# legend-exp/LegendDSP.jl

Measured on NVIDIA B200. Metric: waveforms/sec for dsp_icpc (8192-sample), higher is better.
Workload: dtype f64

## Files before the change

legenddsp.jl_b200/csrc/lgdsp_icpc_split.cuh:

```cuda

constexpr int TTG_LEN = TT_LEN;
constexpr int AUX_LEN = 16;
enum { AX_M = 0, AX_EMAX = 1, AX_YMAX = 2, AX_THR = 3 , AX_POS = 8 , AX_BAD = 13  };

enum { K1R_BLS = 0, K1R_BLSS, K1R_BLSX, K1R_MX , K1R_MN, K1R_SLEN, K1R_SS, K1R_SQ,
       K1R_TLS, K1R_TLSS, K1R_TLSX, K1R_TLBAD, K1R_YMAX, K1R_N };

constexpr int K1_XS = 0;
constexpr int K1_MASK = K1_XS + 2 * MAXN * 2;
constexpr int K1_RED = K1_MASK + 5 * NWORDS * 4;
constexpr int K1_IRED = K1_MASK;
constexpr int K1_BAR = K1_RED + K1R_N * NWARP * 8;
constexpr int TILE_LD = 9;
constexpr int K1_TILE = K1_BAR + 16;
constexpr int K1_TOTAL = K1_TILE + NWARP * 32 * TILE_LD * 8;
static_assert(4 * (K1_TOTAL + 1024) <= 233472, "four CTAs per SM");

template <typename SAMPLE, unsigned GMASK>
__global__ void __launch_bounds__(NT, 4)
icpc_prefix_kernel(const __grid_constant__ IcpcDev P, const SAMPLE* __restrict__ wf, long long n_events, long long ld,
                   const double* __restrict__ bl_ext, long long bl_stride, double bl_div, double* __restrict__ ttg,
                   double* __restrict__ auxg, double* __restrict__ rows)
{
    extern __shared__ __align__(128) unsigned char smem[];
// ... 271 lines not shown
                    uint32_t word = (uint32_t)(mbt << lane);
                    if (lane > 0) word |= (uint32_t)(up >> (33 - lane));
                    uint32_t* M = masks + t * NWORDS;
                    const int w = (CH * wid) + lane;
                    if (w < NWORDS) M[w] = word;
                    if (lane == 31 && w + 1 < NWORDS) M[w + 1] = (uint32_t)(mbt >> 1);
                }
            }
            const double ya = wmax_d(cvalid > 0 ? fmax(fabs(ylo), fabs(yhi)) : 0.0);
            red_put(red, K1R_YMAX, wid, lane, ya);
        }
        {
            double tl_S = 0, tl_SS = 0, tl_SX = 0;
            bool bad = lean;
            double cref = 0.0, cinv = 0.0, clog = 0.0;
            const int ntail = P.tail_until - P.tail_from + 1;
            const int q = lean ? 0 : (ntail + NT - 1) / NT;
            const int ia = P.tail_from + tid * q, ib = min(ia + q - 1, P.tail_until);
            int wcat = 3;
            double c_run = 0.0, cinv_run = 0.0;
            int xref = 0;
            if (q > 0) {
                const int mfl = (int)floor(fmin(fmax(m, -2.0e9), 2.0e9));
                int dmx = 0;
                bool nonpos = false;
                xref = ia <= ib ? (int)xs[ia] : 0;
#pragma unroll 2
                for (int idx = ia; idx <= ib; ++idx) {
                    const int xv = (int)xs[idx];
                    nonpos |= xv <= mfl;
                    dmx = max(dmx, abs(xv - xref));
                }
                int cat = 0;
                if (ia <= ib) {
                    c_run = u2d((uint32_t)xref) - m;
                    cinv_run = 1.0 / c_run;
                    const double au = (double)dmx * cinv_run;
                    cat = (nonpos || !(c_run > 0.0) || au > 0.125) ? 3 : (au > 0.015625 ? 2 : (au > 0.0009765625 ? 1 : 0));
                }
                wcat = __reduce_max_sync(FULL, cat);
            }
            if (wcat < 3) {
                const double clog_run = ia <= ib ? log_d(c_run) : 0.0;
#pragma unroll 1
                for (int idx = ia; idx <= ib; ++idx) {
                    const double u = (double)((int)xs[idx] - xref) * cinv_run;
                    double lg;
                    if (wcat == 0) {
                        double pl = fma(u, 1.0 / 5.0, -1.0 / 4.0);
                        pl = fma(u, pl, 1.0 / 3.0); pl = fma(u, pl, -1.0 / 2.0); pl = fma(u, pl, 1.0);
                        lg = fma(u, pl, clog_run);
                    } else if (wcat == 1) {
                        const double u2 = u * u, u4 = u2 * u2;
                        const double a0 = fma(-1.0 / 2.0, u, 1.0), a1 = fma(-1.0 / 4.0, u, 1.0 / 3.0), a2 = fma(-1.0 / 6.0, u, 1.0 / 5.0),
                                     a3 = fma(-1.0 / 8.0, u, 1.0 / 7.0);
                        const double b0 = fma(a1, u2, a0), b1 = fma(a3, u2, a2);
                        const double c0 = fma(b1, u4, b0);
                        lg = fma(u, fma(u4 * u4, 1.0 / 9.0, c0), clog_run);
                    } else {
                        lg = clog_run + log1p_small(u);
                    }
                    const double X = t_first + (double)idx * dt;
                    tl_S += lg;
                    tl_SS = fma(lg, lg, tl_SS);
                    tl_SX = fma(X, lg, tl_SX);
                }
            } else {
#pragma unroll 1
                for (int i = 0; i < q; ++i) {
                    const int idx = ia + i;
                    const bool act = idx <= ib;
                    const double w = act ? u2d(xs[idx]) - m : cref;
                    const bool pos = w > 0.0;
                    if (act && !pos) bad = true;
                    const double u = (w - cref) * cinv, au = fabs(u);
                    const bool use = act && pos;
                    int cat = 0;
                    if (use) cat = !(cref > 0.0) || au > 0.125 ? 3 : (au > 0.015625 ? 2 : (au > 0.0009765625 ? 1 : 0));
                    const int wcat = __reduce_max_sync(FULL, cat);
                    double lg;
                    if (wcat == 0) {
                        double pl = fma(u, 1.0 / 5.0, -1.0 / 4.0);
                        pl = fma(u, pl, 1.0 / 3.0); pl = fma(u, pl, -1.0 / 2.0); pl = fma(u, pl, 1.0);
                        lg = fma(u, pl, clog);
                    } else if (wcat == 1) {
                        const double u2 = u * u, u4 = u2 * u2;
                        const double a0 = fma(-1.0 / 2.0, u, 1.0), a1 = fma(-1.0 / 4.0, u, 1.0 / 3.0), a2 = fma(-1.0 / 6.0, u, 1.0 / 5.0),
                                     a3 = fma(-1.0 / 8.0, u, 1.0 / 7.0);
                        const double b0 = fma(a1, u2, a0), b1 = fma(a3, u2, a2);
                        const double c0 = fma(b1, u4, b0);
                        lg = fma(u, fma(u4 * u4, 1.0 / 9.0, c0), clog);
                    } else {
                        lg = clog + log1p_small(u);
                        if (cat == 3) {
                            lg = log_d(w);
                            cref = w; cinv = 1.0 / w; clog = lg;
                        }
                    }
                    if (use) {
                        const double X = t_first + (double)idx * dt;
                        tl_S += lg;
                        tl_SS = fma(lg, lg, tl_SS);
                        tl_SX = fma(X, lg, tl_SX);
                    }
                }
            }
            tl_S = wsum_d(tl_S); tl_SS = wsum_d(tl_SS); tl_SX = wsum_d(tl_SX);
            const bool anybad = __any_sync(FULL, bad);
            if (lane == 0) {
                red[K1R_TLS * NWARP + wid] = tl_S; red[K1R_TLSS * NWARP + wid] = tl_SS;
                red[K1R_TLSX * NWARP + wid] = tl_SX; red[K1R_TLBAD * NWARP + wid] = anybad ? 1.0 : 0.0;
            }
        }
        __syncthreads();

        double* ax = auxg + e * AUX_LEN;
        double* ro = rows + e * LGDSP_NCOL;
        if (wid < 5) {
            int pos = -1, mult = 0;
            if ((G & LGDSP_GROUP_TIMING) && !(lean && wid != 1)) resolve_runs(masks + wid * NWORDS, P.tx_min_n, lane, pos, mult);
            if (lane == 0) { ax[AX_POS + wid] = (double)pos; ax[AX_THR + wid] = thr[wid == 0 ? 0 : wid == 1 ? 1 : wid == 2 ? 2 : wid == 3 ? 3 : 4]; }
        } else if (wid == 5) {
            const double blS = red_sum(red, K1R_BLS), blSS = red_sum(red, K1R_BLSS), blSX = red_sum(red, K1R_BLSX);
            const double tlS = red_sum(red, K1R_TLS), tlSS = red_sum(red, K1R_TLSS), tlSX = red_sum(red, K1R_TLSX);
            const double tlbad = red_sum(red, K1R_TLBAD);
            if (lane < 2) {
                const double sY = lane == 0 ? blS : tlS;
                const double sYY = lane == 0 ? blSS : tlSS;
                const double sXY = lane == 0 ? t_first * blS + dt * blSX : tlSX;
                const Stats st = stats_finalize(lane == 0 ? P.bl_inv_n : P.tail_inv_n, lane == 0 ? P.bl_sX : P.tail_sX,
                                                lane == 0 ? P.bl_sXX : P.tail_sXX, sY, sYY, sXY);
                const double bad = wrapped ? CUDART_NAN : 0.0;
                if (lane == 0) {
                    ro[LGDSP_COL_blmean] = st.mean + bad; ro[LGDSP_COL_blsigma] = st.sigma + bad;
                    ro[LGDSP_COL_blslope] = st.slope + bad; ro[LGDSP_COL_bloffset] = st.offset + bad;
                    ro[LGDSP_COL_qc_label] = -1.0 + bad;
                    ro[LGDSP_COL_e_max] = e_max + bad; ro[LGDSP_COL_e_min] = e_min + bad;
                    ro[LGDSP_COL_n_sat_low] = (double)nlow + bad; ro[LGDSP_COL_n_sat_high] = (double)nhigh + bad;
                    ro[LGDSP_COL_n_sat_low_cons] = (double)cons_low + bad; ro[LGDSP_COL_n_sat_high_cons] = (double)cons_high + bad;
                } else {
                    const bool ok = tlbad == 0.0;
                    ro[LGDSP_COL_tail_mean] = (ok ? st.mean : 0.0) + bad; ro[LGDSP_COL_tail_sigma] = (ok ? st.sigma : 0.0) + bad;
                    ro[LGDSP_COL_tail_tau] = (ok ? div_rn(-1.0, st.slope) : 0.0) + bad;
                }
            }
        } else if (wid == 6) {
            const double Ymax = red_max(red, K1R_YMAX);
            if (lane == 0) { ax[AX_M] = m; ax[AX_EMAX] = e_max; ax[AX_YMAX] = Ymax; ax[AX_BAD] = wrapped ? 1.0 : 0.0; }
        }
        __syncthreads();
    }
}

constexpr int NT2 = 256;
constexpr int NW2 = NT2 / 32;
static_assert(NT2 == NT && NW2 == NWARP, "the extract kernel shares the block-reduction helpers and the 33-sample chunking");
enum { MK_T0 = 0, MK_T0INV, MK_CUR, MK_PILE, MK_N };
enum { K2R_PZS = 0, K2R_PZSS, K2R_PZSX, K2R_E104, K2R_E104N, K2R_E313, K2R_E313N, K2R_C535, K2R_CET, K2R_SGMAX, K2R_SGS, K2R_SGSS,
       K2R_CMAX0, K2R_CMAX1, K2R_CMAX2, K2R_CMAX3, K2R_CARG0, K2R_CARG1, K2R_CARG2, K2R_CARG3, K2R_E535, K2R_ETMAX, K2R_ETARG, K2R_N };
constexpr int K2_NTYPE = 5;
constexpr int K2_TT = 0;
constexpr int K2_MASK = K2_TT + TT_LEN * 8;
constexpr int K2_RED = K2_MASK + MK_N * NWORDS * 4;
constexpr int K2_STASH = K2_RED + K2R_N * NW2 * 8;
constexpr int K2_ROW = K2_STASH + LGDSP_MAX_DNI * 8;
constexpr int K2_AUX = K2_ROW + 64 * 8;
constexpr int K2_SGG = K2_AUX + AUX_LEN * 8;
constexpr int K2_FLAG = K2_SGG + 24 * 8;
constexpr int K2_BAR = K2_FLAG + NT2;
constexpr int K2_TOTAL = K2_BAR + 16;
static_assert(3 * (K2_TOTAL + 1024) <= 233472, "three CTAs per SM");

template <unsigned GMASK>
__global__ void __launch_bounds__(NT2, 3)
icpc_extract_kernel(const __grid_constant__ IcpcDev P, const double* __restrict__ ttg, const double* __restrict__ auxg,
                    long long n_events, int write_cz_zeros, double* __restrict__ rows)
{
    extern __shared__ __align__(128) unsigned char smem[];
    double* TT = reinterpret_cast<double*>(smem + K2_TT);
    uint32_t* masks = reinterpret_cast<uint32_t*>(smem + K2_MASK);
    double* red = reinterpret_cast<double*>(smem + K2_RED);
    double* stash = reinterpret_cast<double*>(smem + K2_STASH);
    double* row = reinterpret_cast<double*>(smem + K2_ROW);
    double* aux = reinterpret_cast<double*>(smem + K2_AUX);
    double (*sgg)[8] = reinterpret_cast<double (*)[8]>(smem + K2_SGG);
    unsigned char* flagb = smem + K2_FLAG;
    uint64_t* bar = reinterpret_cast<uint64_t*>(smem + K2_BAR);

    const int tid = threadIdx.x, lane = tid & 31, wid = tid >> 5;
    const int n = P.n;
    const uint32_t tt_bytes = (uint32_t)(n + 2) * 8u;
    const double t_first = P.t_first, dt = P.dt;
    const unsigned G = GMASK ? GMASK : P.groups;
    const double* A_int = P.dni_A;
    const double* A_sig = P.dni_A + LGDSP_MAX_DNI * 4;

    if (tid == 0) {
        mbar_init(bar, 1);
        fence_mbar_init();
    }
    if (tid < TT_LEN - 2 - n) TT[n + 2 + tid] = 0.0;
    if (tid < 24) sgg[tid >> 3][tid & 7] = P.sg[tid >> 3].gg[tid & 7];
    __syncthreads();
    auto sg_at = [&](int f, int j) -> double {
        return (P.sg[f].n_taps + 1 <= 8) ? sg_eval8(TT, sgg[f], j) : sg_eval(TT, P.sg[f].gg, P.sg[f].n_taps, j);
    };
    const int i0 = tid * CH;
    const int nsg = P.sg[0].nout;
    const bool want_cur = (G & LGDSP_GROUP_CURRENT) != 0, want_intr = (G & LGDSP_GROUP_INTRACE) != 0;

    uint32_t it = 0;
    for (long long e = blockIdx.x; e < n_events; e += gridDim.x, ++it) {
        if (tid == 0) {
            fence_proxy_async();
            mbar_expect_tx(bar, tt_bytes);
            tma_load_1d(TT, ttg + e * TTG_LEN, tt_bytes, bar);
            if (e + gridDim.x < n_events) tma_prefetch_l2(ttg + (e + gridDim.x) * TTG_LEN, tt_bytes);
        }
#pragma unroll
        for (int q = 0; q < MK_N; ++q) masks[q * NWORDS + tid] = 0u;
        if (tid < AUX_LEN) aux[tid] = auxg[e * AUX_LEN + tid];
        mbar_wait(bar, it & 1u);

        const bool lean = (G & LGDSP_GROUP_LEAN) != 0;
        const TrapDev& T5 = lean ? P.e10410 : P.e535;
        if (!lean) {
            double pz_S = 0, pz_SS = 0, pz_SX = 0;
#pragma unroll 2
            for (int idx = P.tail_from + tid; idx <= P.tail_until; idx += NT2) {
                const double y = TT[idx + 1] - TT[idx];
                const double X = t_first + (double)idx * dt;
                pz_S += y;
                pz_SS = fma(y, y, pz_SS);
                pz_SX = fma(X, y, pz_SX);
            }
            pz_S = wsum_d(pz_S); pz_SS = wsum_d(pz_SS); pz_SX = wsum_d(pz_SX);
            if (lane == 0) {
                red[K2R_PZS * NW2 + wid] = pz_S; red[K2R_PZSS * NW2 + wid] = pz_SS; red[K2R_PZSX * NW2 + wid] = pz_SX;
            }
        }
        if (!lean && (G & LGDSP_GROUP_TRAPS)) {
            double o4[4];
            trap_full2_minmax(TT, P.e10410, P.e313, tid, o4);
            const double a = wmax_d(o4[0]), b = wmax_d(o4[1]), c = wmax_d(o4[2]), d = wmax_d(o4[3]);
            if (lane == 0) {
                red[K2R_E104 * NW2 + wid] = a; red[K2R_E104N * NW2 + wid] = b;
                red[K2R_E313 * NW2 + wid] = c; red[K2R_E313N * NW2 + wid] = d;
            }
        }
        double c0a = 0, c0b = 0, cia = 0, cib = 0, c5a = -CUDART_INF, c5b = -CUDART_INF, cea = -CUDART_INF, ceb = -CUDART_INF;
        {
            const int ja = i0, jb = i0 + CH;
            if (G & LGDSP_GROUP_TIMING) {
                if (ja < P.t0.nout) c0a = trap_at_i(TT, P.t0, ja);
                if (jb < P.t0.nout) c0b = trap_at_i(TT, P.t0, jb);
                if (!P.t0inv_same && !lean) {
                    if (ja < P.t0inv.nout) cia = trap_at_i(TT, P.t0inv, ja);
                    if (jb < P.t0inv.nout) cib = trap_at_i(TT, P.t0inv, jb);
                }
            }
            if (G & LGDSP_GROUP_TRAPS) {
                if (ja < T5.nout) c5a = trap_at_i(TT, T5, ja);
                if (jb < T5.nout) c5b = trap_at_i(TT, T5, jb);
                const double w5 = wmax_d(c5a);
                red_put(red, K2R_C535, wid, lane, w5);
                if (!lean) {
                    if (ja < P.etrap.nout) cea = trap_at_i(TT, P.etrap, ja);
                    if (jb < P.etrap.nout) ceb = trap_at_i(TT, P.etrap, jb);
                    const double we = wmax_d(cea);
                    red_put(red, K2R_CET, wid, lane, we);
                }
            }
        }
        double sgcmax = -CUDART_INF;
        if (want_cur || want_intr) {
            double cmax[4] = {-CUDART_INF, -CUDART_INF, -CUDART_INF, -CUDART_INF};
            int carg[4] = {0x7fffffff, 0x7fffffff, 0x7fffffff, 0x7fffffff};
            double sg_S = 0, sg_SS = 0;
            if (want_intr) sg_chunk(TT, P.sg[0], i0, min(CH, nsg - i0), [&](int k, double s) { sgcmax = s > sgcmax ? s : sgcmax; });
#pragma unroll 1
            for (int f = 0; f < 3; ++f) {
                if (f > 0 && P.sg_alias[f] >= 0) continue;
                if (f > 0 && !want_cur) continue;
                double bm = -CUDART_INF;
                int ba = 0x7fffffff;
                if (P.sg[f].n_taps + 1 <= 8) {
                    double g[8];
#pragma unroll
                    for (int q = 0; q < 8; ++q) g[q] = sgg[f][q];
                    auto ev = [&](int j) -> double {
                        const double* p = TT + j;
                        double a0 = g[0] * p[0], a1 = g[1] * p[1];
                        a0 = fma(g[2], p[2], a0); a1 = fma(g[3], p[3], a1);
                        a0 = fma(g[4], p[4], a0); a1 = fma(g[5], p[5], a1);
                        a0 = fma(g[6], p[6], a0); a1 = fma(g[7], p[7], a1);
                        return a0 + a1;
                    };
                    if (want_cur) {
#pragma unroll 2
                        for (int j = P.cur_from[f] + tid; j <= P.cur_until[f]; j += NT2) {
                            const double v = ev(j);
                            if (v > bm) { bm = v; ba = j; }
                        }
                    }
                    if (f == 0 && want_intr) {
#pragma unroll 2
                        for (int j = P.intr_from + tid; j <= P.intr_until; j += NT2) {
                            const double v = ev(j);
                            sg_S += v;
                            sg_SS = fma(v, v, sg_SS);
                        }
                    }
                } else {
                    if (want_cur) {
#pragma unroll 1
                        for (int j = P.cur_from[f] + tid; j <= P.cur_until[f]; j += NT2) {
                            const double v = sg_at(f, j);
                            if (v > bm) { bm = v; ba = j; }
                        }
                    }
                    if (f == 0 && want_intr) {
#pragma unroll 1
                        for (int j = P.intr_from + tid; j <= P.intr_until; j += NT2) {
                            const double v = sg_at(0, j);
                            sg_S += v;
                            sg_SS = fma(v, v, sg_SS);
                        }
                    }
                }
                if (f == 0) { cmax[0] = bm; carg[0] = ba; } else if (f == 1) { cmax[1] = bm; carg[1] = ba; } else { cmax[2] = bm; carg[2] = ba; }
            }
            if (want_cur) {
#pragma unroll 2
                for (int j = P.cur_from[3] + tid; j <= P.cur_until[3]; j += NT2) {
                    const double d = deriv_at(TT, j);
                    if (d > cmax[3]) { cmax[3] = d; carg[3] = j; }
                }
            }
            const double wsm = wmax_d(sgcmax);
            sg_S = wsum_d(sg_S); sg_SS = wsum_d(sg_SS);
#pragma unroll
            for (int f = 0; f < 4; ++f) cmax[f] = wargmax_d(cmax[f], carg[f]);
            if (lane == 0) {
                red[K2R_SGMAX * NW2 + wid] = wsm; red[K2R_SGS * NW2 + wid] = sg_S; red[K2R_SGSS * NW2 + wid] = sg_SS;
#pragma unroll
                for (int f = 0; f < 4; ++f) {
                    red[(K2R_CMAX0 + f) * NW2 + wid] = cmax[f];
                    red[(K2R_CARG0 + f) * NW2 + wid] = (double)carg[f];
                }
            }
        }
        __syncthreads();

        if (tid < 64) row[tid] = 0.0;
        const double thr50 = aux[AX_THR + 1];
        const double Ymax = aux[AX_YMAX];
        const double kslack = 1e-7 * Ymax;
        auto tx_us = [&](int k) -> double {
            const int pos = (int)aux[AX_POS + k];
            const double th = aux[AX_THR + k];
            double t = 0.0;
            if (pos >= 1) t = cross_x(th, y_at(TT, pos - 1), y_at(TT, pos), t_first + (double)(pos - 1) * dt, dt) * 0.001;
            return t != t ? 0.0 : t;
        };
        double pk_p;
        int pk_from;
        {
            double t50_us = 0.0;
            const int pos = (int)aux[AX_POS + 1];
            if (pos >= 1) {
                const double x = cross_x(thr50, y_at(TT, pos - 1), y_at(TT, pos), t_first + (double)(pos - 1) * dt, dt);
                t50_us = x * 0.001;
            }
            const double tf = t_first + (double)(P.etrap.L - 1) * dt;
            dni_window(P.sig_dni.n_w, n - P.etrap.L + 1, (t50_us * 1000.0 + P.trap_pick - tf) / dt, pk_p, pk_from);
        }
        if ((G & LGDSP_GROUP_TRAPS) && tid < P.sig_dni.n_w) stash[tid] = trap_at_i(TT, P.etrap, pk_from + tid);

        double pile_thr = 0.0, cur_thr = 0.0;
        if (G & LGDSP_GROUP_INTRACE) {
            cur_thr = red_max(red, K2R_SGMAX) * 0.5;
            const double sS = red_sum(red, K2R_SGS), sSS = red_sum(red, K2R_SGSS);
            const double mean_Y = mul_rn(sS, P.intr_inv_n);
            double var_Y = sub_rn(mul_rn(sSS, P.intr_inv_n), mul_rn(mean_Y, mean_Y));
            if (var_Y < 0) var_Y = 0;
            pile_thr = sqrt(var_Y) * P.nsigma;
            if (pile_thr == 0.0) pile_thr = 1.0;
        }
        double e535 = c5a, etmax = cea;
        int etarg = (cea > -CUDART_INF) ? i0 : 0x7fffffff;
        auto do_item = [&](int type, int q) {
            if (type <= 1) {
                const TrapDev& tr = type == 0 ? P.t0 : P.t0inv;
                const double th = P.t0_thr;
                const int j = q * CH + 1 + lane;
                const bool v = j < tr.nout;
                const double o = v ? trap_at_i(TT, tr, j) : 0.0;
                const unsigned mp = __ballot_sync(FULL, v && (o >= th));
                const unsigned mn_ = __ballot_sync(FULL, v && (-o >= th));
                commit_pair(type == 0 ? masks + MK_T0 * NWORDS : nullptr, (unsigned long long)mp << 1,
                            ((type == 1 || P.t0inv_same) && !lean) ? masks + MK_T0INV * NWORDS : nullptr, (unsigned long long)mn_ << 1,
                            false, 0, q, lane);
            } else if (type == 2) {
                const int j = q * CH + 1 + lane;
                if (j < T5.nout) {
                    const double o = trap_at_i(TT, T5, j);
                    e535 = o > e535 ? o : e535;
                }
            } else if (type == 3) {
                const int j = q * CH + 1 + lane;
                if (j < P.etrap.nout) {
                    const double o = trap_at_i(TT, P.etrap, j);
                    if (o > etmax || (o == etmax && j < etarg)) { etmax = o; etarg = j; }
                }
            } else {
                const int j = q * CH + lane;
                const bool v = j < nsg;
                const double sv = v ? sg_at(0, j) : 0.0;
                const int j2 = q * CH + 32;
                const double s2 = (j2 < nsg) ? sg_at(0, j2) : -CUDART_INF;
                const unsigned long long bc = (unsigned long long)__ballot_sync(FULL, v && (sv >= cur_thr)) |
                                              ((s2 >= cur_thr) ? (1ull << 32) : 0ull);
                const unsigned long long bp = (unsigned long long)__ballot_sync(FULL, v && (sv >= pile_thr)) |
                                              ((s2 >= pile_thr) ? (1ull << 32) : 0ull);
                commit_pair(masks + MK_CUR * NWORDS, bc, masks + MK_PILE * NWORDS, bp, true, nsg, q, lane);
            }
        };
        unsigned flags = 0;
        {
            bool f0 = false, fi = false, f5 = false, fe = false;
            if (G & LGDSP_GROUP_TIMING) {
                const double th = P.t0_thr;
                const int rule = P.t0_min_n >= 2 * CH ? 2 : (P.t0_min_n > CH ? 1 : 0);
                auto need = [&](bool a, bool b, bool valid) -> bool {
                    bool prev = __shfl_up_sync(FULL, a, 1), next = __shfl_down_sync(FULL, b, 1);
                    if (lane == 0) prev = true;
                    if (lane == 31) next = true;
                    if (!valid) return false;
                    return rule == 2 ? ((a && b) || (a && prev) || (b && next)) : (rule == 1 ? (a || b) : true);
                };
                {
                    const bool va = i0 < P.t0.nout, vb = i0 + CH < P.t0.nout;
                    const bool pa = va && (c0a >= th), pb = vb && (c0b >= th);
                    const bool na = va && (-c0a >= th), nb = vb && (-c0b >= th);
                    const bool fp = need(pa, pb, va), fn = need(na, nb, va);
                    f0 = (P.t0inv_same && !lean) ? (fp || fn) : fp;
                    if (pa) mask_commit(masks + MK_T0 * NWORDS, tid, 1ull);
                    if (P.t0inv_same && na && !lean) mask_commit(masks + MK_T0INV * NWORDS, tid, 1ull);
                }
                if (!P.t0inv_same && !lean) {
                    const bool wa = i0 < P.t0inv.nout, wb = i0 + CH < P.t0inv.nout;
                    const bool na = wa && (-cia >= th), nb = wb && (-cib >= th);
                    fi = need(na, nb, wa);
                    if (na) mask_commit(masks + MK_T0INV * NWORDS, tid, 1ull);
                }
            }
            if (G & LGDSP_GROUP_TRAPS) {
                const double M5 = red_max(red, K2R_C535);
                const double k5 = Ymax * 2.0 * (T5.inv1 + T5.inv2) * 1.000001;
                if (i0 + 1 < T5.nout) f5 = interval_bound(c5a, c5b, i0 + CH < T5.nout, k5) + kslack >= M5;
                if (!lean) {
                    const double Me = red_max(red, K2R_CET);
                    const double ke = Ymax * 2.0 * (P.etrap.inv1 + P.etrap.inv2) * 1.000001;
                    if (i0 + 1 < P.etrap.nout) fe = interval_bound(cea, ceb, i0 + CH < P.etrap.nout, ke) + kslack >= Me;
                }
            }
            flags = (f0 ? 1u : 0u) | (fi ? 2u : 0u) | (f5 ? 4u : 0u) | (fe ? 8u : 0u);
        }
        if (G & LGDSP_GROUP_INTRACE) {
            const bool flag = sgcmax >= fmin(cur_thr, pile_thr);
            const unsigned bf = __ballot_sync(FULL, flag);
            if (__popc(bf) > 10) {
                if (flag) {
                    unsigned long long bc = 0, bp = 0;
                    sg_chunk(TT, P.sg[0], i0, min(CH, nsg - i0), [&](int k, double s) {
                        bc |= (s >= cur_thr) ? (1ull << k) : 0ull;
                        bp |= (s >= pile_thr) ? (1ull << k) : 0ull;
                    });
                    mask_commit(masks + MK_CUR * NWORDS, tid, bc);
                    mask_commit_reversed(masks + MK_PILE * NWORDS, tid, bp, nsg);
                }
            } else if (flag) {
                flags |= 16u;
            }
        }
        flagb[tid] = (unsigned char)flags;
        __syncthreads();
        {
            const unsigned myf = flagb[NW2 * lane + wid];
#pragma unroll 1
            for (int type = 0; type < K2_NTYPE; ++type) {
                unsigned word = __ballot_sync(FULL, (myf >> type) & 1u);
                while (word) {
                    const int bq = __ffs(word) - 1;
                    word &= word - 1;
                    do_item(type, NW2 * bq + wid);
                }
            }
            e535 = wmax_d(e535);
            etmax = wargmax_d(etmax, etarg);
            if (lane == 0) {
                red[K2R_E535 * NW2 + wid] = e535;
                red[K2R_ETMAX * NW2 + wid] = etmax; red[K2R_ETARG * NW2 + wid] = (double)etarg;
            }
        }
        __syncthreads();

        auto t0_us = [&](bool inv, int pos) -> double {
            const TrapDev& tr = inv ? P.t0inv : P.t0;
            double t = 0.0;
            if (pos >= 1) {
                const double tl = t_first + (double)(pos - 1 + tr.L - 1) * dt;
                const double sgn = inv ? -1.0 : 1.0;
                t = cross_x(P.t0_thr, sgn * trap_at_i(TT, tr, pos - 1), sgn * trap_at_i(TT, tr, pos), tl, dt) * 0.001;
            }
            return t != t ? 0.0 : t;
        };
        auto qdrift_warp = [&](double t_us, double first, double last) -> double {
            const double tns = t_us * 1000.0;
            if (P.int_dni.n_w <= 8) {
                const int g = lane >> 3;
                const double ts = g == 0 ? tns : (g == 1 ? tns + first : tns + last);
                double pc;
                int from;
                dni_window(P.int_dni.n_w, n, (ts - t_first) / dt, pc, from);
                const double r = dni3_warp(A_int, P.int_dni.n_w, P.int_dni.m, TT + 1, from, pc - (double)from, lane);
                const double a0 = __shfl_sync(FULL, r, 0), a1 = __shfl_sync(FULL, r, 8), a2 = __shfl_sync(FULL, r, 16);
                return (a2 - a1) - (a1 - a0);
            }
            double a[3];
#pragma unroll 1
            for (int q = 0; q < 3; ++q) {
                const double ts = q == 0 ? tns : (q == 1 ? tns + first : tns + last);
                double pc;
                int from;
                dni_window(P.int_dni.n_w, n, (ts - t_first) / dt, pc, from);
                a[q] = dni_eval_warp(A_int, P.int_dni.n_w, P.int_dni.m, TT + from + 1, pc - (double)from, lane);
            }
            const double area1 = a[1] - a[0], area2 = a[2] - a[1];
            return area2 - area1;
        };
        if (wid == 0 && !lean) {
            const double pzS = red_sum(red, K2R_PZS), pzSS = red_sum(red, K2R_PZSS), pzSX = red_sum(red, K2R_PZSX);
            if (lane == 0) {
                const Stats st = stats_finalize(P.tail_inv_n, P.tail_sX, P.tail_sXX, pzS, pzSS, pzSX);
                row[LGDSP_COL_tailmean] = st.mean; row[LGDSP_COL_tailsigma] = st.sigma;
                row[LGDSP_COL_tailslope] = st.slope; row[LGDSP_COL_tailoffset] = st.offset;
            }
            if (G & LGDSP_GROUP_TIMING) {
                int pos0i, mult_;
                resolve_runs(masks + MK_T0INV * NWORDS, P.t0_min_n, lane, pos0i, mult_);
                if (lane == 0) row[LGDSP_COL_t0_inv] = t0_us(true, pos0i);
            }
        } else if (wid == 1) {
            int pos0, mult_;
            resolve_runs(masks + MK_T0 * NWORDS, P.t0_min_n, lane, pos0, mult_);
            double t = 0.0;
            if (lane < 5) {
                t = tx_us(lane);
                if (G & LGDSP_GROUP_TIMING) row[LGDSP_COL_t10 + lane] = t;
            } else if (lane == 5) {
                t = t0_us(false, pos0);
                if (G & LGDSP_GROUP_TIMING) row[LGDSP_COL_t0] = t;
            }
            const double t90 = __shfl_sync(FULL, t, 3), t0v = __shfl_sync(FULL, t, 5);
            if (lane == 0 && (G & LGDSP_GROUP_TIMING)) row[LGDSP_COL_drift_time] = (t90 - t0v) * 1000.0;
        } else if (wid == 2) {
            if (G & LGDSP_GROUP_TRAPS) {
                const double v = dni_eval_warp(A_sig, P.sig_dni.n_w, P.sig_dni.m, stash, pk_p - (double)pk_from, lane);
                if (lean) {
                    const double a = red_max(red, K2R_E535);
                    if (lane == 0) { row[LGDSP_COL_e_10410] = a; row[LGDSP_COL_e_trap] = v; }
                }
                double em = 0;
                int ea = 0;
                if (!lean) red_argmax(red, K2R_ETMAX, K2R_ETARG, em, ea);
                const double a = lean ? 0.0 : red_max(red, K2R_E104), b = lean ? 0.0 : red_max(red, K2R_E535), c = lean ? 0.0 : red_max(red, K2R_E313);
                const double d = lean ? 0.0 : red_max(red, K2R_E104N), f = lean ? 0.0 : red_max(red, K2R_E313N);
                if (lane == 0 && !lean) {
                    row[LGDSP_COL_e_10410] = a; row[LGDSP_COL_e_535] = b; row[LGDSP_COL_e_313] = c;
                    row[LGDSP_COL_e_10410_inv] = d; row[LGDSP_COL_e_313_inv] = f;
                    row[LGDSP_COL_e_trap_max] = em;
                    row[LGDSP_COL_t_trap_max] = t_first + (double)(ea + P.etrap.L - 1) * dt;
                    row[LGDSP_COL_e_trap] = v;
                }
            }
        } else if (wid == 3) {
            if (G & LGDSP_GROUP_CURRENT) {
                double vv[4];
                int aa[4];
#pragma unroll
                for (int f = 0; f < 4; ++f) {
                    const int fs = (f < 3 && P.sg_alias[f] >= 0) ? P.sg_alias[f] : f;
                    red_argmax(red, K2R_CMAX0 + fs, K2R_CARG0 + fs, vv[f], aa[f]);
                }
                if (lane < 4) {
                    const int f = lane;
                    double v = f == 0 ? vv[0] : f == 1 ? vv[1] : f == 2 ? vv[2] : vv[3];
                    const int a = f == 0 ? aa[0] : f == 1 ? aa[1] : f == 2 ? aa[2] : aa[3];
                    if (a > P.cur_from[f] && a < P.cur_until[f]) {
                        const double y1 = (f < 3) ? sg_at(f, a - 1) : deriv_at(TT, a - 1);
                        const double y3 = (f < 3) ? sg_at(f, a + 1) : deriv_at(TT, a + 1);
                        v = extrema3(y1, v, y3);
                    }
                    row[LGDSP_COL_a_sg + f] = v;
                }
            }
        } else if (wid == 4) {
            if (G & LGDSP_GROUP_INTRACE) {
                int posc, multc;
                resolve_runs(masks + MK_CUR * NWORDS, P.tx_min_n, lane, posc, multc);
                if (lane == 0) {
                    const double tf = t_first + (double)P.sg[0].offset * dt;
                    double t = 0.0;
                    if (posc >= 1) {
                        t = cross_x(cur_thr, sg_at(0, posc - 1), sg_at(0, posc), tf + (double)(posc - 1) * dt, dt) * 0.001;
                        if (t != t) t = 0.0;
                    }
                    row[LGDSP_COL_t50_current] = t;
                }
            }
        } else if (wid == 5) {
            if (G & LGDSP_GROUP_INTRACE) {
                int posp, multp;
                resolve_runs(masks + MK_PILE * NWORDS, P.intr_min_n, lane, posp, multp);
                if (lane == 0) {
                    const double tf = t_first + (double)P.sg[0].offset * dt;
                    double xi = CUDART_NAN;
                    if (posp >= 1) {
                        const double yl = sg_at(0, nsg - 1 - (posp - 1)), yr = sg_at(0, nsg - 1 - posp);
                        xi = cross_x(pile_thr, yl, yr, tf + (double)(posp - 1) * dt, dt);
                    }
                    const double last_t = tf + (double)(nsg - 1) * dt;
                    row[LGDSP_COL_inTrace_intersect] = last_t - xi;
                    row[LGDSP_COL_inTrace_n] = (double)multp;
                }
            }
        } else if (wid == 7) {
            if (G & LGDSP_GROUP_QDRIFT) {
                int pos0, mult_;
                resolve_runs(masks + MK_T0 * NWORDS, P.t0_min_n, lane, pos0, mult_);
                const double v = qdrift_warp(t0_us(false, pos0), P.qd_first, P.qd_last);
                if (lane == 0) row[LGDSP_COL_qdrift] = v;
            }
        } else if (wid == 6) {
            if (G & LGDSP_GROUP_QDRIFT) {
                const double v = qdrift_warp(tx_us(2), P.lq_first, P.lq_last);
                if (lane == 0) row[LGDSP_COL_lq] = v;
            }
        }
        __syncthreads();
        if (tid < LGDSP_NCOL) {
            const bool k1col = tid <= LGDSP_COL_bloffset || tid == LGDSP_COL_qc_label ||
                               (tid >= LGDSP_COL_tail_tau && tid <= LGDSP_COL_e_min) || tid >= LGDSP_COL_n_sat_low;
            const bool k3col = tid == LGDSP_COL_e_cusp || tid == LGDSP_COL_e_zac || tid == LGDSP_COL_e_cusp_max ||
                               tid == LGDSP_COL_e_zac_max || tid == LGDSP_COL_t_cusp_max || tid == LGDSP_COL_t_zac_max;
            if (!k1col && (!k3col || write_cz_zeros)) rows[e * LGDSP_NCOL + tid] = aux[AX_BAD] != 0.0 ? CUDART_NAN : row[tid];
        }
    }
}

constexpr int CZ_REC = 12;
constexpr int CZ_MAXC = NT;
constexpr int CZ_HDR = 16;
enum { CZH_N = 0, CZH_MAXC, CZH_ARGC, CZH_MAXZ, CZH_ARGZ, CZH_PKP0, CZH_PKF0, CZH_PKP1, CZH_PKF1,
       CZH_CNT };
constexpr int CZP_LEN = CZ_HDR + CZ_MAXC * CZ_REC;
constexpr int K4_NBLK = 4;
constexpr int CZ_SCR = K4_NBLK * 4 + 2 * LGDSP_MAX_DNI;
constexpr int CZG_LEN = 2 * CZP_LEN + CZ_SCR;

enum { K3R_CZC0 = 0, K3R_CZC1, K3R_CZMAX0, K3R_CZARG0, K3R_CZMAX1, K3R_CZARG1, K3R_CZSCR, K3R_CZSCR1, K3R_CZSCR2, K3R_CZSCR3, K3R_N };
enum { K3I_CZN = 0, K3I_PKFROM = 1 , K3I_N = 4 };
constexpr int K3_TT = 0;
constexpr int K3_TABA = K3_TT + TT_LEN * 8;
constexpr int K3_TABB = K3_TABA + 8 * NT * 8;
constexpr int K3_CZCO = K3_TABB + 8 * NT * 8;
constexpr int K3_RED = K3_CZCO + 2 * NT * 8;
constexpr int K3_STASH = K3_RED + K3R_N * NWARP * 8;
constexpr int K3_SCR = K3_STASH + 2 * LGDSP_MAX_DNI * 8;
constexpr int K3_IBUF = K3_SCR + 8 * 8;
constexpr int K3_BAR = K3_IBUF + K3I_N * 4;
constexpr int K3_PAR = K3_BAR + 16;
constexpr int K3_TOTAL = K3_PAR + (int)sizeof(SmemPar);
static_assert(2 * (K3_TOTAL + 1024) <= 233472, "two CTAs per SM");
enum { K3S_PKP = 0 , K3S_PP0 = 2, K3S_YMAX = 3 };

template <typename TC, typename TA, typename TD>
__device__ __forceinline__ void cz_select(const CzDev& Z, const double* TT, int n, int nw, double pp0, double Ymax, const int* pk_from,
                                          const double* pk_p, bool want_cusp, bool want_zac, double* czco, double* red, int* czn,
                                          double* cg, TC&& tab_c, TA&& tab_a, TD&& tt_dead)
{
    const int tid = threadIdx.x, lane = tid & 31, wid = tid >> 5;
    const int i0 = tid * CH;
    CzState st;
    st.active = false;
    double oc = -CUDART_INF, oz = -CUDART_INF;
    cz_init_with(Z, TT, n, tid, pp0, st, tab_c, tab_a);
    cz_coarse(Z, TT, n, tid, st, oc, oz);
    if (!want_cusp) oc = -CUDART_INF;
    if (!want_zac) oz = -CUDART_INF;
    const int j0 = i0 - Z.L + 1;
    czco[tid] = oc;
    czco[NT + tid] = oz;
    {
        int ac = oc > -CUDART_INF ? j0 : 0x7fffffff, az = oz > -CUDART_INF ? j0 : 0x7fffffff;
        const double wc = wargmax_d(oc, ac), wz = wargmax_d(oz, az);
        if (lane == 0) {
            red[K3R_CZMAX0 * NWARP + wid] = wc; red[K3R_CZARG0 * NWARP + wid] = (double)ac;
            red[K3R_CZMAX1 * NWARP + wid] = wz; red[K3R_CZARG1 * NWARP + wid] = (double)az;
        }
    }
    __syncthreads();
    tt_dead();
    double Mc, Mz;
    int Ac, Az;
    red_argmax(red, K3R_CZMAX0, K3R_CZARG0, Mc, Ac);
    red_argmax(red, K3R_CZMAX1, K3R_CZARG1, Mz, Az);
    bool cand = false;
    if (st.active) {
        const int t1 = min(tid + 1, NT - 1);
        const double kap = Ymax * 1.000001;
        const int jlo = i0 - Z.L + 1, jhi = jlo + CH - 1;
        if (want_cusp) {
            const double a = oc, b = (tid + 1 < NT) ? czco[t1] : -CUDART_INF;
            const double kc = kap * Z.lip_cusp;
            double bound;
            if (a > -CUDART_INF) bound = interval_bound(a, b, b > -CUDART_INF, kc);
            else if (b > -CUDART_INF) bound = fma((double)CH, kc, b);
            else bound = CUDART_INF;
// ... 308 lines not shown
```

Before: 7.220 million.

## Double extract kernel block to 512 threads with specialized helper warp half

The extract kernel now launches 512 threads. The first 256 keep the per-chunk work: tail stats, intrace SG stats, derivative argmax, timing and flag building. The second 256 take the independent full-range passes: trap min/max, the SG current-filter argmaxes and the energy stash. The aim is to shorten per-event latency by running these sweeps concurrently within one CTA, and the late per-type stage reductions use 16 warps through a separate red16 buffer. The cost is two CTAs per SM instead of three, plus more complex indexing for the reduction slots.

```diff
diff --git a/legenddsp.jl_b200/csrc/lgdsp_icpc_split.cuh b/legenddsp.jl_b200/csrc/lgdsp_icpc_split.cuh
--- a/legenddsp.jl_b200/csrc/lgdsp_icpc_split.cuh
+++ b/legenddsp.jl_b200/csrc/lgdsp_icpc_split.cuh
@@ -447,27 +447,37 @@
     }
 }
 
-constexpr int NT2 = 256;
+constexpr int NT2 = 512;
 constexpr int NW2 = NT2 / 32;
-static_assert(NT2 == NT && NW2 == NWARP, "the extract kernel shares the block-reduction helpers and the 33-sample chunking");
+static_assert(NT2 == 2 * NT, "warps 8..15 mirror the owners' thread indices (tid - NT)");
 enum { MK_T0 = 0, MK_T0INV, MK_CUR, MK_PILE, MK_N };
 enum { K2R_PZS = 0, K2R_PZSS, K2R_PZSX, K2R_E104, K2R_E104N, K2R_E313, K2R_E313N, K2R_C535, K2R_CET, K2R_SGMAX, K2R_SGS, K2R_SGSS,
-       K2R_CMAX0, K2R_CMAX1, K2R_CMAX2, K2R_CMAX3, K2R_CARG0, K2R_CARG1, K2R_CARG2, K2R_CARG3, K2R_E535, K2R_ETMAX, K2R_ETARG, K2R_N };
+       K2R_CMAX0, K2R_CMAX1, K2R_CMAX2, K2R_CMAX3, K2R_CARG0, K2R_CARG1, K2R_CARG2, K2R_CARG3, K2R_N };
+enum { K2Q_E535 = 0, K2Q_ETMAX, K2Q_ETARG, K2Q_N };
 constexpr int K2_NTYPE = 5;
 constexpr int K2_TT = 0;
 constexpr int K2_MASK = K2_TT + TT_LEN * 8;
 constexpr int K2_RED = K2_MASK + MK_N * NWORDS * 4;
-constexpr int K2_STASH = K2_RED + K2R_N * NW2 * 8;
+constexpr int K2_RED16 = K2_RED + K2R_N * NWARP * 8;
+constexpr int K2_STASH = K2_RED16 + K2Q_N * NW2 * 8;
 constexpr int K2_ROW = K2_STASH + LGDSP_MAX_DNI * 8;
 constexpr int K2_AUX = K2_ROW + 64 * 8;
 constexpr int K2_SGG = K2_AUX + AUX_LEN * 8;
 constexpr int K2_FLAG = K2_SGG + 24 * 8;
-constexpr int K2_BAR = K2_FLAG + NT2;
+constexpr int K2_BAR = K2_FLAG + NT;
 constexpr int K2_TOTAL = K2_BAR + 16;
-static_assert(3 * (K2_TOTAL + 1024) <= 233472, "three CTAs per SM");
+static_assert(2 * (K2_TOTAL + 1024) <= 233472, "two CTAs per SM");
+
+__device__ __forceinline__ double red16_max(const double* red16, int slot) { return wmax_d(red16[slot * NW2 + (threadIdx.x & 15)]); }
+__device__ __forceinline__ void red16_argmax(const double* red16, int slot_v, int slot_i, double& v, int& ix)
+{
+    int pi = (int)red16[slot_i * NW2 + (threadIdx.x & 15)];
+    v = wargmax_d(red16[slot_v * NW2 + (threadIdx.x & 15)], pi);
+    ix = pi;
+}
 
 template <unsigned GMASK>
-__global__ void __launch_bounds__(NT2, 3)
+__global__ void __launch_bounds__(NT2, 2)
 icpc_extract_kernel(const __grid_constant__ IcpcDev P, const double* __restrict__ ttg, const double* __restrict__ auxg,
                     long long n_events, int write_cz_zeros, double* __restrict__ rows)
 {
@@ -475,6 +485,7 @@
     double* TT = reinterpret_cast<double*>(smem + K2_TT);
     uint32_t* masks = reinterpret_cast<uint32_t*>(smem + K2_MASK);
     double* red = reinterpret_cast<double*>(smem + K2_RED);
+    double* red16 = reinterpret_cast<double*>(smem + K2_RED16);
     double* stash = reinterpret_cast<double*>(smem + K2_STASH);
     double* row = reinterpret_cast<double*>(smem + K2_ROW);
     double* aux = reinterpret_cast<double*>(smem + K2_AUX);
@@ -483,6 +494,8 @@
     uint64_t* bar = reinterpret_cast<uint64_t*>(smem + K2_BAR);
 
     const int tid = threadIdx.x, lane = tid & 31, wid = tid >> 5;
+    const bool owner = tid < NT;
+    const int ht = tid & (NT - 1), hw = wid & (NWARP - 1);
     const int n = P.n;
     const uint32_t tt_bytes = (uint32_t)(n + 2) * 8u;
     const double t_first = P.t_first, dt = P.dt;
@@ -512,39 +525,71 @@
             tma_load_1d(TT, ttg + e * TTG_LEN, tt_bytes, bar);
             if (e + gridDim.x < n_events) tma_prefetch_l2(ttg + (e + gridDim.x) * TTG_LEN, tt_bytes);
         }
+        static_assert(MK_N * NWORDS % NT2 == 0, "mask clearing");
 #pragma unroll
-        for (int q = 0; q < MK_N; ++q) masks[q * NWORDS + tid] = 0u;
+        for (int q = 0; q < MK_N * NWORDS / NT2; ++q) masks[q * NT2 + tid] = 0u;
         if (tid < AUX_LEN) aux[tid] = auxg[e * AUX_LEN + tid];
         mbar_wait(bar, it & 1u);
 
         const bool lean = (G & LGDSP_GROUP_LEAN) != 0;
         const TrapDev& T5 = lean ? P.e10410 : P.e535;
-        if (!lean) {
-            double pz_S = 0, pz_SS = 0, pz_SX = 0;
+        double c0a = 0, c0b = 0, cia = 0, cib = 0, c5a = -CUDART_INF, c5b = -CUDART_INF, cea = -CUDART_INF, ceb = -CUDART_INF;
+        double sgcmax = -CUDART_INF;
+        if (owner) {
+            if (!lean) {
+                double pz_S = 0, pz_SS = 0, pz_SX = 0;
 #pragma unroll 2
-            for (int idx = P.tail_from + tid; idx <= P.tail_until; idx += NT2) {
-                const double y = TT[idx + 1] - TT[idx];
-                const double X = t_first + (double)idx * dt;
-                pz_S += y;
-                pz_SS = fma(y, y, pz_SS);
-                pz_SX = fma(X, y, pz_SX);
-            }
-            pz_S = wsum_d(pz_S); pz_SS = wsum_d(pz_SS); pz_SX = wsum_d(pz_SX);
-            if (lane == 0) {
-                red[K2R_PZS * NW2 + wid] = pz_S; red[K2R_PZSS * NW2 + wid] = pz_SS; red[K2R_PZSX * NW2 + wid] = pz_SX;
-            }
-        }
-        if (!lean && (G & LGDSP_GROUP_TRAPS)) {
-            double o4[4];
-            trap_full2_minmax(TT, P.e10410, P.e313, tid, o4);
-            const double a = wmax_d(o4[0]), b = wmax_d(o4[1]), c = wmax_d(o4[2]), d = wmax_d(o4[3]);
-            if (lane == 0) {
-                red[K2R_E104 * NW2 + wid] = a; red[K2R_E104N * NW2 + wid] = b;
-                red[K2R_E313 * NW2 + wid] = c; red[K2R_E313N * NW2 + wid] = d;
-            }
-        }
-        double c0a = 0, c0b = 0, cia = 0, cib = 0, c5a = -CUDART_INF, c5b = -CUDART_INF, cea = -CUDART_INF, ceb = -CUDART_INF;
-        {
+                for (int idx = P.tail_from + tid; idx <= P.tail_until; idx += NT) {
+                    const double y = TT[idx + 1] - TT[idx];
+                    const double X = t_first + (double)idx * dt;
+                    pz_S += y;
+                    pz_SS = fma(y, y, pz_SS);
+                    pz_SX = fma(X, y, pz_SX);
+                }
+                pz_S = wsum_d(pz_S); pz_SS = wsum_d(pz_SS); pz_SX = wsum_d(pz_SX);
+                if (lane == 0) {
+                    red[K2R_PZS * NWARP + wid] = pz_S; red[K2R_PZSS * NWARP + wid] = pz_SS; red[K2R_PZSX * NWARP + wid] = pz_SX;
+                }
+            }
+            if (want_intr) {
+                sg_chunk(TT, P.sg[0], i0, min(CH, nsg - i0), [&](int k, double s) { sgcmax = s > sgcmax ? s : sgcmax; });
+                double sg_S = 0, sg_SS = 0;
+                if (P.sg[0].n_taps + 1 <= 8) {
+#pragma unroll 2
+                    for (int j = P.intr_from + tid; j <= P.intr_until; j += NT) {
+                        const double* p = TT + j;
+                        const double* g = sgg[0];
+                        double a0 = g[0] * p[0], a1 = g[1] * p[1];
+                        a0 = fma(g[2], p[2], a0); a1 = fma(g[3], p[3], a1);
+                        a0 = fma(g[4], p[4], a0); a1 = fma(g[5], p[5], a1);
+                        a0 = fma(g[6], p[6], a0); a1 = fma(g[7], p[7], a1);
+                        const double v = a0 + a1;
+                        sg_S += v;
+                        sg_SS = fma(v, v, sg_SS);
+                    }
+                } else {
+#pragma unroll 1
+                    for (int j = P.intr_from + tid; j <= P.intr_until; j += NT) {
+                        const double v = sg_at(0, j);
+                        sg_S += v;
+                        sg_SS = fma(v, v, sg_SS);
+                    }
+                }
+                const double wsm = wmax_d(sgcmax);
+                sg_S = wsum_d(sg_S); sg_SS = wsum_d(sg_SS);
+                if (lane == 0) { red[K2R_SGMAX * NWARP + wid] = wsm; red[K2R_SGS * NWARP + wid] = sg_S; red[K2R_SGSS * NWARP + wid] = sg_SS; }
+            }
+            if (want_cur) {
+                double dm = -CUDART_INF;
+                int da = 0x7fffffff;
+#pragma unroll 2
+                for (int j = P.cur_from[3] + tid; j <= P.cur_until[3]; j += NT) {
+                    const double d = deriv_at(TT, j);
+                    if (d > dm) { dm = d; da = j; }
+                }
+                dm = wargmax_d(dm, da);
+                if (lane == 0) { red[K2R_CMAX3 * NWARP + wid] = dm; red[K2R_CARG3 * NWARP + wid] = (double)da; }
+            }
             const int ja = i0, jb = i0 + CH;
             if (G & LGDSP_GROUP_TIMING) {
                 if (ja < P.t0.nout) c0a = trap_at_i(TT, P.t0, ja);
@@ -566,82 +611,43 @@
                     red_put(red, K2R_CET, wid, lane, we);
                 }
             }
-        }
-        double sgcmax = -CUDART_INF;
-        if (want_cur || want_intr) {
-            double cmax[4] = {-CUDART_INF, -CUDART_INF, -CUDART_INF, -CUDART_INF};
-            int carg[4] = {0x7fffffff, 0x7fffffff, 0x7fffffff, 0x7fffffff};
-            double sg_S = 0, sg_SS = 0;
-            if (want_intr) sg_chunk(TT, P.sg[0], i0, min(CH, nsg - i0), [&](int k, double s) { sgcmax = s > sgcmax ? s : sgcmax; });
+        } else {
+            if (!lean && (G & LGDSP_GROUP_TRAPS)) {
+                double o4[4];
+                trap_full2_minmax(TT, P.e10410, P.e313, ht, o4);
+                const double a = wmax_d(o4[0]), b = wmax_d(o4[1]), c = wmax_d(o4[2]), d = wmax_d(o4[3]);
+                if (lane == 0) {
+                    red[K2R_E104 * NWARP + hw] = a; red[K2R_E104N * NWARP + hw] = b;
+                    red[K2R_E313 * NWARP + hw] = c; red[K2R_E313N * NWARP + hw] = d;
+                }
+            }
+            if (want_cur) {
 #pragma unroll 1
-            for (int f = 0; f < 3; ++f) {
-                if (f > 0 && P.sg_alias[f] >= 0) continue;
-                if (f > 0 && !want_cur) continue;
-                double bm = -CUDART_INF;
-                int ba = 0x7fffffff;
-                if (P.sg[f].n_taps + 1 <= 8) {
-                    double g[8];
-#pragma unroll
-                    for (int q = 0; q < 8; ++q) g[q] = sgg[f][q];
-                    auto ev = [&](int j) -> double {
-                        const double* p = TT + j;
-                        double a0 = g[0] * p[0], a1 = g[1] * p[1];
-                        a0 = fma(g[2], p[2], a0); a1 = fma(g[3], p[3], a1);
-                        a0 = fma(g[4], p[4], a0); a1 = fma(g[5], p[5], a1);
-                        a0 = fma(g[6], p[6], a0); a1 = fma(g[7], p[7], a1);
-                        return a0 + a1;
-                    };
-                    if (want_cur) {
+                for (int f = 0; f < 3; ++f) {
+                    if (f > 0 && P.sg_alias[f] >= 0) continue;
+                    double bm = -CUDART_INF;
+                    int ba = 0x7fffffff;
+                    if (P.sg[f].n_taps + 1 <= 8) {
+                        const double* g = sgg[f];
 #pragma unroll 2
-                        for (int j = P.cur_from[f] + tid; j <= P.cur_until[f]; j += NT2) {
-                            const double v = ev(j);
+                        for (int j = P.cur_from[f] + ht; j <= P.cur_until[f]; j += NT) {
+                            const double* p = TT + j;
+                            double a0 = g[0] * p[0], a1 = g[1] * p[1];
+                            a0 = fma(g[2], p[2], a0); a1 = fma(g[3], p[3], a1);
+                            a0 = fma(g[4], p[4], a0); a1 = fma(g[5], p[5], a1);
+                            a0 = fma(g[6], p[6], a0); a1 = fma(g[7], p[7], a1);
+                            const double v = a0 + a1;
                             if (v > bm) { bm = v; ba = j; }
                         }
-                    }
-                    if (f == 0 && want_intr) {
-#pragma unroll 2
-                        for (int j = P.intr_from + tid; j <= P.intr_until; j += NT2) {
-                            const double v = ev(j);
-                            sg_S += v;
-                            sg_SS = fma(v, v, sg_SS);
-                        }
-                    }
-                } else {
-                    if (want_cur) {
+                    } else {
 #pragma unroll 1
-                        for (int j = P.cur_from[f] + tid; j <= P.cur_until[f]; j += NT2) {
+                        for (int j = P.cur_from[f] + ht; j <= P.cur_until[f]; j += NT) {
                             const double v = sg_at(f, j);
                             if (v > bm) { bm = v; ba = j; }
                         }
                     }
-                    if (f == 0 && want_intr) {
-#pragma unroll 1
-                        for (int j = P.intr_from + tid; j <= P.intr_until; j += NT2) {
-                            const double v = sg_at(0, j);
-                            sg_S += v;
-                            sg_SS = fma(v, v, sg_SS);
-                        }
-                    }
-                }
-                if (f == 0) { cmax[0] = bm; carg[0] = ba; } else if (f == 1) { cmax[1] = bm; carg[1] = ba; } else { cmax[2] = bm; carg[2] = ba; }
-            }
-            if (want_cur) {
-#pragma unroll 2
-                for (int j = P.cur_from[3] + tid; j <= P.cur_until[3]; j += NT2) {
-                    const double d = deriv_at(TT, j);
-                    if (d > cmax[3]) { cmax[3] = d; carg[3] = j; }
-                }
-            }
-            const double wsm = wmax_d(sgcmax);
-            sg_S = wsum_d(sg_S); sg_SS = wsum_d(sg_SS);
-#pragma unroll
-            for (int f = 0; f < 4; ++f) cmax[f] = wargmax_d(cmax[f], carg[f]);
-            if (lane == 0) {
-                red[K2R_SGMAX * NW2 + wid] = wsm; red[K2R_SGS * NW2 + wid] = sg_S; red[K2R_SGSS * NW2 + wid] = sg_SS;
-#pragma unroll
-                for (int f = 0; f < 4; ++f) {
-                    red[(K2R_CMAX0 + f) * NW2 + wid] = cmax[f];
-                    red[(K2R_CARG0 + f) * NW2 + wid] = (double)carg[f];
+                    bm = wargmax_d(bm, ba);
+                    if (lane == 0) { red[(K2R_CMAX0 + f) * NWARP + hw] = bm; red[(K2R_CARG0 + f) * NWARP + hw] = (double)ba; }
                 }
             }
         }
@@ -670,7 +676,7 @@
             const double tf = t_first + (double)(P.etrap.L - 1) * dt;
             dni_window(P.sig_dni.n_w, n - P.etrap.L + 1, (t50_us * 1000.0 + P.trap_pick - tf) / dt, pk_p, pk_from);
         }
-        if ((G & LGDSP_GROUP_TRAPS) && tid < P.sig_dni.n_w) stash[tid] = trap_at_i(TT, P.etrap, pk_from + tid);
+        if ((G & LGDSP_GROUP_TRAPS) && !owner && ht < P.sig_dni.n_w) stash[ht] = trap_at_i(TT, P.etrap, pk_from + ht);
 
         double pile_thr = 0.0, cur_thr = 0.0;
         if (G & LGDSP_GROUP_INTRACE) {
@@ -722,67 +728,69 @@
             }
         };
         unsigned flags = 0;
-        {
-            bool f0 = false, fi = false, f5 = false, fe = false;
-            if (G & LGDSP_GROUP_TIMING) {
-                const double th = P.t0_thr;
-                const int rule = P.t0_min_n >= 2 * CH ? 2 : (P.t0_min_n > CH ? 1 : 0);
-                auto need = [&](bool a, bool b, bool valid) -> bool {
-                    bool prev = __shfl_up_sync(FULL, a, 1), next = __shfl_down_sync(FULL, b, 1);
-                    if (lane == 0) prev = true;
-                    if (lane == 31) next = true;
-                    if (!valid) return false;
-                    return rule == 2 ? ((a && b) || (a && prev) || (b && next)) : (rule == 1 ? (a || b) : true);
-                };
-                {
-                    const bool va = i0 < P.t0.nout, vb = i0 + CH < P.t0.nout;
-                    const bool pa = va && (c0a >= th), pb = vb && (c0b >= th);
-                    const bool na = va && (-c0a >= th), nb = vb && (-c0b >= th);
-                    const bool fp = need(pa, pb, va), fn = need(na, nb, va);
-                    f0 = (P.t0inv_same && !lean) ? (fp || fn) : fp;
-                    if (pa) mask_commit(masks + MK_T0 * NWORDS, tid, 1ull);
-                    if (P.t0inv_same && na && !lean) mask_commit(masks + MK_T0INV * NWORDS, tid, 1ull);
-                }
-                if (!P.t0inv_same && !lean) {
-                    const bool wa = i0 < P.t0inv.nout, wb = i0 + CH < P.t0inv.nout;
-                    const bool na = wa && (-cia >= th), nb = wb && (-cib >= th);
-                    fi = need(na, nb, wa);
-                    if (na) mask_commit(masks + MK_T0INV * NWORDS, tid, 1ull);
-                }
-            }
-            if (G & LGDSP_GROUP_TRAPS) {
-                const double M5 = red_max(red, K2R_C535);
-                const double k5 = Ymax * 2.0 * (T5.inv1 + T5.inv2) * 1.000001;
-                if (i0 + 1 < T5.nout) f5 = interval_bound(c5a, c5b, i0 + CH < T5.nout, k5) + kslack >= M5;
-                if (!lean) {
-                    const double Me = red_max(red, K2R_CET);
-                    const double ke = Ymax * 2.0 * (P.etrap.inv1 + P.etrap.inv2) * 1.000001;
-                    if (i0 + 1 < P.etrap.nout) fe = interval_bound(cea, ceb, i0 + CH < P.etrap.nout, ke) + kslack >= Me;
-                }
-            }
-            flags = (f0 ? 1u : 0u) | (fi ? 2u : 0u) | (f5 ? 4u : 0u) | (fe ? 8u : 0u);
-        }
-        if (G & LGDSP_GROUP_INTRACE) {
-            const bool flag = sgcmax >= fmin(cur_thr, pile_thr);
-            const unsigned bf = __ballot_sync(FULL, flag);
-            if (__popc(bf) > 10) {
-                if (flag) {
-                    unsigned long long bc = 0, bp = 0;
-                    sg_chunk(TT, P.sg[0], i0, min(CH, nsg - i0), [&](int k, double s) {
-                        bc |= (s >= cur_thr) ? (1ull << k) : 0ull;
-                        bp |= (s >= pile_thr) ? (1ull << k) : 0ull;
-                    });
-                    mask_commit(masks + MK_CUR * NWORDS, tid, bc);
-                    mask_commit_reversed(masks + MK_PILE * NWORDS, tid, bp, nsg);
-                }
-            } else if (flag) {
-                flags |= 16u;
-            }
-        }
-        flagb[tid] = (unsigned char)flags;
+        if (owner) {
+            {
+                bool f0 = false, fi = false, f5 = false, fe = false;
+                if (G & LGDSP_GROUP_TIMING) {
+                    const double th = P.t0_thr;
+                    const int rule = P.t0_min_n >= 2 * CH ? 2 : (P.t0_min_n > CH ? 1 : 0);
+                    auto need = [&](bool a, bool b, bool valid) -> bool {
+                        bool prev = __shfl_up_sync(FULL, a, 1), next = __shfl_down_sync(FULL, b, 1);
+                        if (lane == 0) prev = true;
+                        if (lane == 31) next = true;
+                        if (!valid) return false;
+                        return rule == 2 ? ((a && b) || (a && prev) || (b && next)) : (rule == 1 ? (a || b) : true);
+                    };
+                    {
+                        const bool va = i0 < P.t0.nout, vb = i0 + CH < P.t0.nout;
+                        const bool pa = va && (c0a >= th), pb = vb && (c0b >= th);
+                        const bool na = va && (-c0a >= th), nb = vb && (-c0b >= th);
+                        const bool fp = need(pa, pb, va), fn = need(na, nb, va);
+                        f0 = (P.t0inv_same && !lean) ? (fp || fn) : fp;
+                        if (pa) mask_commit(masks + MK_T0 * NWORDS, tid, 1ull);
+                        if (P.t0inv_same && na && !lean) mask_commit(masks + MK_T0INV * NWORDS, tid, 1ull);
+                    }
+                    if (!P.t0inv_same && !lean) {
+                        const bool wa = i0 < P.t0inv.nout, wb = i0 + CH < P.t0inv.nout;
+                        const bool na = wa && (-cia >= th), nb = wb && (-cib >= th);
+                        fi = need(na, nb, wa);
+                        if (na) mask_commit(masks + MK_T0INV * NWORDS, tid, 1ull);
+                    }
+                }
+                if (G & LGDSP_GROUP_TRAPS) {
+                    const double M5 = red_max(red, K2R_C535);
+                    const double k5 = Ymax * 2.0 * (T5.inv1 + T5.inv2) * 1.000001;
+                    if (i0 + 1 < T5.nout) f5 = interval_bound(c5a, c5b, i0 + CH < T5.nout, k5) + kslack >= M5;
+                    if (!lean) {
+                        const double Me = red_max(red, K2R_CET);
+                        const double ke = Ymax * 2.0 * (P.etrap.inv1 + P.etrap.inv2) * 1.000001;
+                        if (i0 + 1 < P.etrap.nout) fe = interval_bound(cea, ceb, i0 + CH < P.etrap.nout, ke) + kslack >= Me;
+                    }
+                }
+                flags = (f0 ? 1u : 0u) | (fi ? 2u : 0u) | (f5 ? 4u : 0u) | (fe ? 8u : 0u);
+            }
+            if (G & LGDSP_GROUP_INTRACE) {
+                const bool flag = sgcmax >= fmin(cur_thr, pile_thr);
+                const unsigned bf = __ballot_sync(FULL, flag);
+                if (__popc(bf) > 10) {
+                    if (flag) {
+                        unsigned long long bc = 0, bp = 0;
+                        sg_chunk(TT, P.sg[0], i0, min(CH, nsg - i0), [&](int k, double s) {
+                            bc |= (s >= cur_thr) ? (1ull << k) : 0ull;
+                            bp |= (s >= pile_thr) ? (1ull << k) : 0ull;
+                        });
+                        mask_commit(masks + MK_CUR * NWORDS, tid, bc);
+                        mask_commit_reversed(masks + MK_PILE * NWORDS, tid, bp, nsg);
+                    }
+                } else if (flag) {
+                    flags |= 16u;
+                }
+            }
+        }
+        if (owner) flagb[tid] = (unsigned char)flags;
         __syncthreads();
         {
-            const unsigned myf = flagb[NW2 * lane + wid];
+            const unsigned myf = lane < NT / NW2 ? flagb[NW2 * lane + wid] : 0u;
 #pragma unroll 1
             for (int type = 0; type < K2_NTYPE; ++type) {
                 unsigned word = __ballot_sync(FULL, (myf >> type) & 1u);
@@ -795,8 +803,8 @@
             e535 = wmax_d(e535);
             etmax = wargmax_d(etmax, etarg);
             if (lane == 0) {
-                red[K2R_E535 * NW2 + wid] = e535;
-                red[K2R_ETMAX * NW2 + wid] = etmax; red[K2R_ETARG * NW2 + wid] = (double)etarg;
+                red16[K2Q_E535 * NW2 + wid] = e535;
+                red16[K2Q_ETMAX * NW2 + wid] = etmax; red16[K2Q_ETARG * NW2 + wid] = (double)etarg;
             }
         }
         __syncthreads();
@@ -835,17 +843,20 @@
             const double area1 = a[1] - a[0], area2 = a[2] - a[1];
             return area2 - area1;
         };
-        if (wid == 0 && !lean) {
-            const double pzS = red_sum(red, K2R_PZS), pzSS = red_sum(red, K2R_PZSS), pzSX = red_sum(red, K2R_PZSX);
-            if (lane == 0) {
-                const Stats st = stats_finalize(P.tail_inv_n, P.tail_sX, P.tail_sXX, pzS, pzSS, pzSX);
-                row[LGDSP_COL_tailmean] = st.mean; row[LGDSP_COL_tailsigma] = st.sigma;
-                row[LGDSP_COL_tailslope] = st.slope; row[LGDSP_COL_tailoffset] = st.offset;
-            }
-            if (G & LGDSP_GROUP_TIMING) {
+        if (wid == 0) {
+            if ((G & LGDSP_GROUP_TIMING) && !lean) {
                 int pos0i, mult_;
                 resolve_runs(masks + MK_T0INV * NWORDS, P.t0_min_n, lane, pos0i, mult_);
                 if (lane == 0) row[LGDSP_COL_t0_inv] = t0_us(true, pos0i);
+            }
+        } else if (wid == 8) {
+            if (!lean) {
+                const double pzS = red_sum(red, K2R_PZS), pzSS = red_sum(red, K2R_PZSS), pzSX = red_sum(red, K2R_PZSX);
+                if (lane == 0) {
+                    const Stats st = stats_finalize(P.tail_inv_n, P.tail_sX, P.tail_sXX, pzS, pzSS, pzSX);
+                    row[LGDSP_COL_tailmean] = st.mean; row[LGDSP_COL_tailsigma] = st.sigma;
+                    row[LGDSP_COL_tailslope] = st.slope; row[LGDSP_COL_tailoffset] = st.offset;
+                }
             }
         } else if (wid == 1) {
             int pos0, mult_;
@@ -864,13 +875,13 @@
             if (G & LGDSP_GROUP_TRAPS) {
                 const double v = dni_eval_warp(A_sig, P.sig_dni.n_w, P.sig_dni.m, stash, pk_p - (double)pk_from, lane);
                 if (lean) {
-                    const double a = red_max(red, K2R_E535);
+                    const double a = red16_max(red16, K2Q_E535);
                     if (lane == 0) { row[LGDSP_COL_e_10410] = a; row[LGDSP_COL_e_trap] = v; }
                 }
                 double em = 0;
                 int ea = 0;
-                if (!lean) red_argmax(red, K2R_ETMAX, K2R_ETARG, em, ea);
-                const double a = lean ? 0.0 : red_max(red, K2R_E104), b = lean ? 0.0 : red_max(red, K2R_E535), c = lean ? 0.0 : red_max(red, K2R_E313);
+                if (!lean) red16_argmax(red16, K2Q_ETMAX, K2Q_ETARG, em, ea);
+                const double a = lean ? 0.0 : red_max(red, K2R_E104), b = lean ? 0.0 : red16_max(red16, K2Q_E535), c = lean ? 0.0 : red_max(red, K2R_E313);
                 const double d = lean ? 0.0 : red_max(red, K2R_E104N), f = lean ? 0.0 : red_max(red, K2R_E313N);
                 if (lane == 0 && !lean) {
                     row[LGDSP_COL_e_10410] = a; row[LGDSP_COL_e_535] = b; row[LGDSP_COL_e_313] = c;
```

Result: slower. 6.933 million, median of 6 (-4.0%).
